# tungphambasement/TNN

Measured on AMD Instinct MI355X. Metric: images/sec (whole node) WRN-16-8 on 32x32x3, pipeline-parallel, higher is better.
Workload: dtype bf16; 1 GPU; model=cifar100_wrn16_8, global_batch=256, input=32x32x3, microbatches=1, graphed_step=True, parallelism=single

## Files before the change

tnn_amd/csrc/bindings.cpp:

```cpp

#include <array>
#include <torch/extension.h>
#include <ATen/hip/HIPContext.h>

#include "kernels.h"

namespace tnn {

static hipStream_t cur_stream() {
  return at::hip::getCurrentHIPStreamMasqueradingAsCUDA().stream();
}

static void* zero_page(const at::Tensor& like) {
  static at::Tensor z;
  if (!z.defined() || z.device() != like.device())
    z = at::zeros({16}, like.options().dtype(at::kFloat));
  return z.data_ptr();
}

static DT dt_of(const at::Tensor& t) {
  if (t.scalar_type() == at::kFloat) return DT::F32;
  if (t.scalar_type() == at::kBFloat16) return DT::BF16;
  TORCH_CHECK(false, "tnn_amd kernels support fp32/bf16, got ", t.scalar_type());
}
// ... 431 lines not shown
at::Tensor conv2d_dgrad(const at::Tensor& dy, const at::Tensor& w, int64_t H,
                        int64_t W, int64_t sh, int64_t sw, int64_t ph,
                        int64_t pw) {
  CHECK_IN(dy);
  CHECK_IN(w);
  int KH = w.size(0), KW = w.size(1), Cin = w.size(2), Cout = w.size(3);
  auto cs = conv_shape_out(dy.size(0), H, W, Cin, Cout, KH, KW, sh, sw, ph, pw,
                           dy.size(1), dy.size(2));
  auto dx = at::empty({cs.N, H, W, Cin}, dy.options());
  if (conv2d_dgrad_wants_db(dt_of(dy), dy.data_ptr(), cs)) {
    auto w_t2d = at::empty({Cin, (int64_t)KH * KW * Cout}, w.options());
    transpose_w_dgrad_launch(dt_of(w), w.data_ptr(), w_t2d.data_ptr(), KH * KW,
                             Cin, Cout, cur_stream());
    conv2d_dgrad_launch(dt_of(dy), dy.data_ptr(), nullptr, w_t2d.data_ptr(),
                        dx.data_ptr(), zero_page(dy), cs, cur_stream());
    return dx;
  }
  auto w_t = at::empty({KH, KW, Cout, Cin}, w.options());
  transpose_w_launch(dt_of(w), w.data_ptr(), w_t.data_ptr(), KH, KW, Cin, Cout,
                     cur_stream());
  conv2d_dgrad_launch(dt_of(dy), dy.data_ptr(), w_t.data_ptr(), nullptr,
                      dx.data_ptr(), zero_page(dy), cs, cur_stream());
  return dx;
}

static at::Tensor conv2d_wgrad_rows(const at::Tensor& x, const at::Tensor& dy,
                                    int64_t KH, int64_t KW, int64_t sh,
                                    int64_t sw, int64_t ph, int64_t pw,
                                    bool out_in_dt, bool bias) {
  CHECK_IN(x);
  CHECK_IN(dy);
  auto cs = conv_shape(x, x.size(3), dy.size(3), KH, KW, sh, sw, ph, pw);
  TORCH_CHECK(dy.size(1) == cs.OH && dy.size(2) == cs.OW, "wgrad shape");
  DT out_dt = out_in_dt ? dt_of(x) : DT::F32;
  const int64_t rows = KH * KW * cs.Cin + (bias ? 1 : 0);
  auto out = at::empty({rows, (int64_t)cs.Cout},
                       out_dt == DT::F32 ? x.options().dtype(at::kFloat)
                                         : x.options());
  int z = conv2d_wgrad_zsplits(cs);
  at::Tensor ws;
  float* wsp = nullptr;
  if (z > 1 || out_dt != DT::F32) {
    ws = at::empty({(int64_t)z * rows * cs.Cout},
                   x.options().dtype(at::kFloat));
    wsp = ws.data_ptr<float>();
  }
// ... 852 lines not shown
  m.def("relu_bwd_mask", &tnn::relu_bwd_mask);
  m.def("add_act_fwd", &tnn::add_act_fwd);
  m.def("add_act_bwd", &tnn::add_act_bwd);
  m.def("dropout_fwd", &tnn::dropout_fwd, py::arg("x"), py::arg("p"),
        py::arg("seed"), py::arg("ctr") = c10::nullopt);
  m.def("dropout_bwd", &tnn::dropout_bwd);
  m.def("colsum", &tnn::colsum);
  m.def("gemm", &tnn::gemm, py::arg("a"), py::arg("b"), py::arg("bias"),
        py::arg("act_kind"), py::arg("residual") = c10::nullopt,
        py::arg("ln_gamma") = c10::nullopt, py::arg("ln_beta") = c10::nullopt,
        py::arg("ln_eps") = 1e-5);
  m.def("gemm_skinny", &tnn::gemm_skinny, py::arg("a"), py::arg("b"),
        py::arg("bias"), py::arg("act_kind"),
        py::arg("residual") = c10::nullopt, py::arg("ln_gamma") = c10::nullopt,
        py::arg("ln_beta") = c10::nullopt, py::arg("ln_eps") = 1e-5);
  m.def("skinny_enabled", &tnn::skinny_enabled);
  m.def("gemm_nt", &tnn::gemm_nt);
  m.def("gemm_tn", &tnn::gemm_tn);
  m.def("mfma_selftest", &tnn::mfma_selftest);
  m.def("mfma_selftest_f32", &tnn::mfma_selftest_f32);
  m.def("conv2d_fwd", &tnn::conv2d_fwd);
  m.def("conv2d_fwd_stats", &tnn::conv2d_fwd_stats);
  m.def("conv2d_dgrad", &tnn::conv2d_dgrad);
  m.def("conv2d_wgrad", &tnn::conv2d_wgrad);
  m.def("conv2d_wgrad_bias", &tnn::conv2d_wgrad_bias);
  m.def("bn_fwd_train", &tnn::bn_fwd_train, py::arg("x"), py::arg("gamma"),
        py::arg("beta"), py::arg("rmean"), py::arg("rvar"),
        py::arg("momentum"), py::arg("eps"), py::arg("relu"),
        py::arg("dropout_p"), py::arg("seed"), py::arg("precomp"),
        py::arg("ctr") = c10::nullopt);
  m.def("bn_fwd_infer", &tnn::bn_fwd_infer);
  m.def("bn_bwd", &tnn::bn_bwd, py::arg("x"), py::arg("dy"),
        py::arg("gamma"), py::arg("mean"), py::arg("invstd"),
        py::arg("y_relu"), py::arg("dy_scale"),
        py::arg("resid") = py::none());
  m.def("maxpool_fwd", &tnn::maxpool_fwd);
  m.def("maxpool_bwd", &tnn::maxpool_bwd);
  m.def("avgpool_fwd", &tnn::avgpool_fwd);
  m.def("avgpool_bwd", &tnn::avgpool_bwd);
  m.def("ce_fwd", &tnn::ce_fwd);
  m.def("ce_bwd", &tnn::ce_bwd);
  m.def("ptloss_fwd", &tnn::ptloss_fwd);
  m.def("ptloss_bwd", &tnn::ptloss_bwd);
  m.def("gn_fwd", &tnn::gn_fwd);
  m.def("gn_bwd", &tnn::gn_bwd);
  m.def("ln_fwd", &tnn::ln_fwd);
// ... 46 lines not shown
```

tnn_amd/csrc/conv2d.hip:

```cpp

#include "common.h"
#include "kernels.h"
#include "tile_gemm.h"

namespace tnn {

using namespace tile;

template <bool POW2>
DEV int idiv(int x, const IDiv& f) {
  if constexpr (POW2) return x >> f.lg;
  else if (f.magic)
    return (int)(((unsigned long long)(unsigned)x * f.magic) >> f.sh);
  else
    return x / f.d;
}
template <bool POW2>
DEV int imod(int x, const IDiv& f) {
  if constexpr (POW2) return x & (f.d - 1);
  else return x - idiv<POW2>(x, f) * f.d;
}

DEV void kdecode(int kidx, const ConvShape& cs, int& kh, int& kw) {
  kh = (kidx * cs.mkw16) >> 16;
// ... 134 lines not shown
    Pack16<T> v = {};
    if (gm < M && gk < K) v = gather(gm, gk);
    *(Pack16<T>*)&As[lds_off<T>(row, kk)] = v;
  }
}
template <typename T, typename RowFn>
DEV void stage_b_transposed(T* Bs, RowFn&& rowptr, int ncols, int n0, int k0,
                            int K) {
  constexpr int V = 16 / sizeof(T);
#pragma unroll
  for (int c = threadIdx.x; c < BK * (BN / V); c += THREADS) {
    int kk = c / (BN / V);
    int nn = (c % (BN / V)) * V;
    int gk = k0 + kk;
    Pack16<T> v = {};
    if (gk < K) v = load16_guarded(rowptr(gk), n0 + nn, ncols);
#pragma unroll
    for (int j = 0; j < V; ++j)
      Bs[lds_off<T>(nn + j, kk)] = v.e[j];
  }
}


template <typename T>
DEV void conv_fwd_store(const WaveCoord& wc, f32x4 acc[FM][FN], const T* bias,
                        T* Y, const ConvShape& cs, int act_kind, int m0,
                        int n0, int M) {
  epilogue_visit(wc, acc, m0, n0, [&](int row, int col, float v) {
    if (row < M && col < cs.Cout) {
      if (bias) v += VecIO<T>::to_f32(bias[col]);
      if (act_kind != ACT_LINEAR) v = act_apply(v, act_kind);
      Y[(int64_t)row * cs.Cout + col] = VecIO<T>::from_f32(v);
    }
  });
}

template <typename T>
DEV void conv_fwd_stats(const WaveCoord& wc, f32x4 acc[FM][FN],
                        const T* bias_p, float* stats, const ConvShape& cs,
                        int m0, int n0, int M) {
  float* ssum = stats;
  float* ssumsq = stats + cs.Cout;
  const int cr = (wc.lane >> 4) * 4;
  const int cc = wc.lane & 15;
#pragma unroll
  for (int fn = 0; fn < FN; ++fn) {
    int col = n0 + wc.wcol0 + fn * 16 + cc;
    float bias = 0.0f;
    if (col < cs.Cout) {
      if (bias_p) bias = VecIO<T>::to_f32(bias_p[col]);
    }
    float s = 0.0f, ss = 0.0f;
#pragma unroll
    for (int fm = 0; fm < FM; ++fm)
#pragma unroll
      for (int j = 0; j < 4; ++j) {
        int row = m0 + wc.wrow0 + fm * 16 + cr + j;
        if (row < M && col < cs.Cout) {
          float v = acc[fm][fn][j] + bias;
          s += v;
          ss += v * v;
        }
      }
    s += __shfl_xor(s, 16, 64);
    ss += __shfl_xor(ss, 16, 64);
    s += __shfl_xor(s, 32, 64);
    ss += __shfl_xor(ss, 32, 64);
    if (wc.lane < 16 && col < cs.Cout) {
      atomicAdd(&ssum[col], s);
      atomicAdd(&ssumsq[col], ss);
    }
  }
}

template <bool POW2, typename T, bool S2>
DEV void dgrad_store(const WaveCoord& wc, f32x4 acc[FM][FN], T* DX,
                     const ConvShape& cs, const DgradClass<S2>& dc, int m0,
                     int n0) {
  epilogue_visit(wc, acc, m0, n0, [&](int row, int col, float v) {
    if (row < dc.M && col < cs.Cin)
      DX[dc.template pixel<POW2>(cs, row) * cs.Cin + col] =
          VecIO<T>::from_f32(v);
  });
}

DEV float* wgrad_slab_store(const WaveCoord& wc, f32x4 acc[FM][FN],
                            float* DW, const ConvShape& cs, int Kout,
                            int bias_row, int r0, int n0) {
  float* out = DW + (int64_t)blockIdx.z * (Kout + bias_row) * cs.Cout;
  epilogue_visit(wc, acc, r0, n0, [&](int row, int col, float v) {
    if (row < Kout && col < cs.Cout) out[(int64_t)row * cs.Cout + col] = v;
  });
  return out;
}
DEV void wgrad_colsum_store(float* out, const ConvShape& cs, int Kout, int n0,
                            float bsum) {
  bsum = colsum_tile_finish(bsum);
  int col = n0 + (threadIdx.x >> 2);
  if ((threadIdx.x & 3) == 0 && col < cs.Cout)
    out[(int64_t)Kout * cs.Cout + col] = bsum;
}

template <bool DB, typename T, typename RowFn, typename TapFn, typename AtFn>
DEV void conv_db_kloop(T* As0, T* As1, T* Bs0, T* Bs1,
                       const WaveCoord& wc, f32x4 acc[FM][FN],
                       const T* __restrict__ asrc, int lgSW, int lgC,
                       const T* __restrict__ bsrc, int64_t bstride,
                       int brows, int m0, int n0, int K,
                       const T* __restrict__ zero16, RowFn&& row,
                       TapFn&& tap, AtFn&& at) {
  constexpr int NA = glds_count<T, BM>();
  constexpr int NB = glds_count<T, BN>();
  constexpr int NPER = NA + NB;
  const int wid = __builtin_amdgcn_readfirstlane(wc.wid);
  const bool uni = lgC >= 6;

  const T* ab[NA];
  int ap[NA], aq[NA];
  const T* bb[NB];
  bool bok[NB];
#pragma unroll
  for (int i = 0; i < NA; ++i) {
    const int j = wid * NA + i;
    int64_t noff;
    int p, q;
    const bool ok = row(m0 + glds_row<T>(j, wc.lane), noff, p, q);
    ab[i] = asrc + noff + (uni ? glds_kk<T>(j, wc.lane) : 0);
    ap[i] = ok ? p : -(1 << 28);
    aq[i] = q;
  }
#pragma unroll
  for (int i = 0; i < NB; ++i) {
    const int j = wid * NB + i;
    const int gn = n0 + glds_row<T>(j, wc.lane);
    bok[i] = gn < brows;
// ... 58 lines not shown
      wait_vmcnt<0>();
    }
    __builtin_amdgcn_s_barrier();
    compute(a_cur, b_cur);
    __builtin_amdgcn_s_barrier();
  };
  if constexpr (DB) {
    stage(0, As0, Bs0);
    for (int t = 0; t < nch; t += 2) {
      step(t, As0, Bs0, As1, Bs1);
      if (t + 1 < nch) step(t + 1, As1, Bs1, As0, Bs0);
    }
  } else {
    for (int t = 0; t < nch; ++t) {
      stage(t, As0, Bs0);
      wait_vmcnt<0>();
      __builtin_amdgcn_s_barrier();
      compute(As0, Bs0);
      __builtin_amdgcn_s_barrier();
    }
  }
}

template <typename T, bool STATS, bool DB>
DEV void conv_fwd_glds_tile(const T* __restrict__ X,
                            const T* __restrict__ WT2,
                            const T* __restrict__ bias, T* __restrict__ Y,
                            const T* __restrict__ zero16, const ConvShape& cs,
                            int act_kind, float* __restrict__ stats) {
  const int M = cs.N * cs.OH * cs.OW;
  const int K = cs.KH * cs.KW * cs.Cin;
  int tm_, tn_;
  conv_tile_order(cs, tm_, tn_);
  const int m0 = tm_ * BM;
  const int n0 = tn_ * BN;
  const WaveCoord wc;
  f32x4 acc[FM][FN] = {};

  auto row = [&](int gm, int64_t& noff, int& p, int& q) {
    const int n = gm >> cs.d_ohow.lg;
    const int rem = gm & (cs.OH * cs.OW - 1);
    p = (rem >> cs.d_ow.lg) * cs.SH - cs.PH;
    q = (rem & (cs.OW - 1)) * cs.SW - cs.PW;
    noff = (int64_t)n << (cs.d_hw.lg + cs.d_cin.lg);
    return gm < M;
  };
  auto tap = [&](int gk, int& dh, int& dw, int& c, int& bcol) {
    kdecode(gk >> cs.d_cin.lg, cs, dh, dw);
    c = gk & (cs.Cin - 1);
    bcol = gk;
  };
  auto at = [&](int p, int q, int dh, int dw, int& ih, int& iw) {
    ih = p + dh;
    iw = q + dw;
    return (unsigned)ih < (unsigned)cs.H && (unsigned)iw < (unsigned)cs.W;
  };
  if constexpr (DB) {
    __shared__ alignas(16) T As0[BM * BK], As1[BM * BK];
    __shared__ alignas(16) T Bs0[BN * BK], Bs1[BN * BK];
    conv_db_kloop<true>(As0, As1, Bs0, Bs1, wc, acc, X, cs.d_w.lg,
                        cs.d_cin.lg, WT2, (int64_t)K, cs.Cout, m0, n0, K,
                        zero16, row, tap, at);
  } else {
    __shared__ alignas(16) T As0[BM * BK], Bs0[BN * BK];
    conv_db_kloop<false>(As0, As0, Bs0, Bs0, wc, acc, X, cs.d_w.lg,
                         cs.d_cin.lg, WT2, (int64_t)K, cs.Cout, m0, n0, K,
                         zero16, row, tap, at);
  }

  conv_fwd_store(wc, acc, bias, Y, cs, act_kind, m0, n0, M);
  if constexpr (STATS) conv_fwd_stats(wc, acc, bias, stats, cs, m0, n0, M);
}

template <typename T, bool STATS = false>
__launch_bounds__(THREADS)
__global__ void k_conv_fwd_db(const T* __restrict__ X,
                              const T* __restrict__ WT2,
                              const T* __restrict__ bias, T* __restrict__ Y,
                              const T* __restrict__ zero16, ConvShape cs,
                              int act_kind, float* __restrict__ stats) {
  conv_fwd_glds_tile<T, STATS, true>(X, WT2, bias, Y, zero16, cs, act_kind,
                                     stats);
}

template <bool STATS>
__launch_bounds__(THREADS)
__global__ void k_conv_fwd_sb(const bf16* __restrict__ X,
                              const bf16* __restrict__ WT2,
                              const bf16* __restrict__ bias,
                              bf16* __restrict__ Y,
                              const bf16* __restrict__ zero16, ConvShape cs,
                              int act_kind, float* __restrict__ stats) {
  conv_fwd_glds_tile<bf16, STATS, false>(X, WT2, bias, Y, zero16, cs, act_kind,
                                         stats);
}

template <typename T, bool POW2, bool GLDS>
__launch_bounds__(THREADS)
__global__ void k_conv_fwd(const T* __restrict__ X, const T* __restrict__ Wt,
                           const T* __restrict__ bias, T* __restrict__ Y,
                           const T* __restrict__ zero16, ConvShape cs,
                           int act_kind) {
  static_assert(!GLDS || POW2, "the LDS-DMA gate implies an all-pow2 shape");
  __shared__ alignas(16) T As[BM * BK];
  __shared__ alignas(16) T Bs[BN * BK];

  const int M = cs.N * cs.OH * cs.OW;
  const int K = cs.KH * cs.KW * cs.Cin;
  int tm_, tn_;
  conv_tile_order(cs, tm_, tn_);
  const int m0 = tm_ * BM;
  const int n0 = tn_ * BN;
  const WaveCoord wc;
  f32x4 acc[FM][FN] = {};

  auto a_src = [&](int k0, int rl, int kk) -> const T* {
    int gm = m0 + rl, gk = k0 + kk;
// ... 68 lines not shown
            if (const T* p = src(gm, gk + j, nullptr)) v.e[j] = *p;
          }
        }
        return v;
      });
    }
    stage_b_transposed(
        Bs,
        [&](int gk) {
          int64_t wrow = gk;
          if constexpr (S2)
            wrow = (int64_t)dc.tap(cs, idiv<POW2>(gk, cs.d_cout)).widx *
                       cs.Cout + imod<POW2>(gk, cs.d_cout);
          return &WT[wrow * cs.Cin];
        },
        cs.Cin, n0, k0, K);
    __syncthreads();
    mfma_compute_tile(As, Bs, wc, acc);
    __syncthreads();
  }
  dgrad_store<POW2>(wc, acc, DX, cs, dc, m0, n0);
}

template <typename T, bool S2 = false, bool S1 = false>
__launch_bounds__(THREADS)
__global__ void k_conv_dgrad_db(const T* __restrict__ DY,
                                const T* __restrict__ WT2D,
                                T* __restrict__ DX,
                                const T* __restrict__ zero16, ConvShape cs) {
  const DgradClass<S2> dc(cs);
  const int M = dc.M, K = dc.K;
  const int KFULL = cs.KH * cs.KW * cs.Cout;
  int tm_, tn_;
  conv_tile_order(cs, tm_, tn_);
  const int m0 = tm_ * BM;
  const int n0 = tn_ * BN;
  const WaveCoord wc;
  f32x4 acc[FM][FN] = {};

  __shared__ alignas(16) T As0[BM * BK], As1[BM * BK];
  __shared__ alignas(16) T Bs0[BN * BK], Bs1[BN * BK];
  conv_db_kloop<true>(
      As0, As1, Bs0, Bs1, wc, acc, DY, cs.d_ow.lg, cs.d_cout.lg, WT2D,
      (int64_t)KFULL, cs.Cin, m0, n0, K, zero16,
      [&](int gm, int64_t& noff, int& p, int& q) {
        const int n = gm >> cs.d_hw.lg;
        const int rem = gm & (dc.Hc * dc.Wc - 1);
        int ih = rem >> cs.d_w.lg, iw = rem & (dc.Wc - 1);
        if constexpr (S2) {
          p = (2 * ih + dc.cls_a + cs.PH - dc.start_h) >> 1;
          q = (2 * iw + dc.cls_b + cs.PW - dc.start_w) >> 1;
        } else {
          p = ih + cs.PH;
          q = iw + cs.PW;
        }
        noff = (int64_t)n << (cs.d_ohow.lg + cs.d_cout.lg);
        return gm < M;
      },
      [&](int gk, int& dh, int& dw, int& c, int& bcol) {
        const int kidx = gk >> cs.d_cout.lg;
        c = gk & (cs.Cout - 1);
        if constexpr (S2) {
          const DgradTap t = dc.tap(cs, kidx);
          dh = t.khi;
          dw = t.kwi;
          bcol = (t.widx << cs.d_cout.lg) + c;
        } else {
          kdecode(kidx, cs, dh, dw);
          bcol = gk;
        }
      },
      [&](int p, int q, int dh, int dw, int& oh, int& ow) {
        const int th = p - dh, tw = q - dw;
        if constexpr (S2 || S1) {
          oh = th;
          ow = tw;
          return (unsigned)oh < (unsigned)cs.OH &&
                 (unsigned)ow < (unsigned)cs.OW;
        } else {
          oh = th / cs.SH;
          ow = tw / cs.SW;
          return th >= 0 && tw >= 0 && oh * cs.SH == th &&
                 ow * cs.SW == tw && oh < cs.OH && ow < cs.OW;
        }
      });
  dgrad_store<true>(wc, acc, DX, cs, dc, m0, n0);
}

template <typename T, bool POW2>
__launch_bounds__(THREADS, 3)
__global__ void k_conv_wgrad(const T* __restrict__ X, const T* __restrict__ DY,
                             float* __restrict__ DW, ConvShape cs,
                             int bias_row) {
  constexpr int V = 16 / sizeof(T);
  __shared__ alignas(16) T As[BM * BK];
  __shared__ alignas(16) T Bs[BN * BK];

  const int M = cs.N * cs.OH * cs.OW;
  const int Kout = cs.KH * cs.KW * cs.Cin;
  int tr_, tn_;
  conv_tile_order(cs, tr_, tn_);
  const int r0 = tr_ * BM;
  const int n0 = tn_ * BN;
  const int m_begin = (int)((int64_t)M * blockIdx.z / gridDim.z);
  const int m_end = (int)((int64_t)M * (blockIdx.z + 1) / gridDim.z);
  const WaveCoord wc;
  f32x4 acc[FM][FN] = {};
  const bool colsum = bias_row && tr_ == 0;
  float bsum = 0.0f;

  for (int k0 = m_begin; k0 < m_end; k0 += BK) {
// ... 274 lines not shown
  return cs.d_ohow.lg >= 0 && cs.d_ow.lg >= 0 && cs.d_cin.lg >= 0 &&
         cs.d_hw.lg >= 0 && cs.d_w.lg >= 0 && cs.d_cout.lg >= 0;
}

static bool vec_ok(DT dt, const void* ptr, int channels) {
  return channels % vec_elems(dt) == 0 && ptr_aligned16(ptr);
}

static int env_int(const char* name, int dflt) {
  const char* e = getenv(name);
  return e ? atoi(e) : dflt;
}

static bool db_on() {
  static const bool on = env_int("TNN_FWD_DB", 1) != 0;
  return on;
}

static int fwd_db_maxk() {
  static const int maxk = env_int("TNN_DB_MAXK", 2304);
  return maxk;
}

template <typename... KArgs, typename... Args>
static void launch(void (*kern)(KArgs...), dim3 grid, hipStream_t s,
                   Args... args) {
  hipLaunchKernelGGL(kern, grid, dim3(THREADS), 0, s, args...);
}

bool conv2d_fwd_wants_db(DT dt, const void* x, const ConvShape& cs) {
  if (!db_on()) return false;
  if (dt == DT::F32 && cs.KH * cs.KW * cs.Cin > fwd_db_maxk()) return false;
  return all_pow2(cs) && vec_ok(dt, x, cs.Cin);
}

static void transpose2d_launch(DT dt, const void* in, void* out, int batch,
                               int rows, int cols, hipStream_t s) {
  dim3 grid((cols + 31) / 32, (rows + 31) / 32, batch);
  dispatch_dt(dt, [&](auto tag) {
    using T = typename decltype(tag)::type;
    hipLaunchKernelGGL(k_transpose2d_tiled<T>, grid, dim3(256), 0, s,
                       (const T*)in, (T*)out, rows, cols);
  });
}

void transpose_w_fwd_launch(DT dt, const void* w, void* w_t2, int KHW, int Cin,
                            int Cout, hipStream_t s) {
  transpose2d_launch(dt, w, w_t2, 1, KHW * Cin, Cout, s);
}

void transpose_w_launch(DT dt, const void* w, void* w_t, int KH, int KW,
                        int Cin, int Cout, hipStream_t s) {
  transpose2d_launch(dt, w, w_t, KH * KW, Cin, Cout, s);
}

void transpose_w_dgrad_launch(DT dt, const void* w, void* w_t2d, int KHW,
                              int Cin, int Cout, hipStream_t s) {
  const bool vec = vec_ok(dt, w, Cout);
  int64_t n = (int64_t)KHW * Cin * (vec ? Cout / vec_elems(dt) : Cout);
  int blocks = (int)((n + 255) / 256);
  dispatch_dt(dt, [&](auto tag) {
    using T = typename decltype(tag)::type;
    auto kern = vec ? k_transpose_w_dgrad_vec<T> : k_transpose_w_dgrad<T>;
    hipLaunchKernelGGL(kern, dim3(blocks), dim3(256), 0, s, (const T*)w,
                       (T*)w_t2d, KHW, Cin, Cout);
  });
}

void conv2d_fwd_launch(DT dt, const void* x, const void* w, const void* w_t2,
                       const void* bias, void* y, const void* zero16,
                       float* stats, const ConvShape& cs, bool relu,
                       hipStream_t s) {
  int M = cs.N * cs.OH * cs.OW;
  dim3 grid(ceil_div(M, BM), ceil_div(cs.Cout, BN));
  int act = relu ? ACT_RELU : ACT_LINEAR;
  bool p2 = all_pow2(cs);
  bool g = p2 && vec_ok(dt, x, cs.Cin);
  dispatch_dt(dt, [&](auto tag) {
    using T = typename decltype(tag)::type;
    auto X = (const T*)x;
    auto B = (const T*)bias;
    auto Y = (T*)y;
    auto Z = (const T*)zero16;
    if (w_t2) {
      if constexpr (sizeof(T) == 2) {
        if (cs.KH * cs.KW * cs.Cin > fwd_db_maxk())
          return launch(stats ? k_conv_fwd_sb<true> : k_conv_fwd_sb<false>,
                        grid, s, X, (const T*)w_t2, B, Y, Z, cs, act, stats);
      }
      return launch(stats ? k_conv_fwd_db<T, true> : k_conv_fwd_db<T, false>,
                    grid, s, X, (const T*)w_t2, B, Y, Z, cs, act, stats);
    }
    launch(g ? k_conv_fwd<T, true, true>
             : (p2 ? k_conv_fwd<T, true, false> : k_conv_fwd<T, false, false>),
           grid, s, X, (const T*)w, B, Y, Z, cs, act);
  });
}

bool conv2d_dgrad_wants_db(DT dt, const void* dy, const ConvShape& cs) {
  if (!db_on()) return false;
  static const int maxk = env_int("TNN_DB_MAXK_DGRAD", 4608);
  return cs.KH * cs.KW * cs.Cout <= maxk && all_pow2(cs) &&
         vec_ok(dt, dy, cs.Cout);
}

void conv2d_dgrad_launch(DT dt, const void* dy, const void* w_t,
                         const void* w_t2d, void* dx, const void* zero16,
                         const ConvShape& cs, hipStream_t s) {
  int M = cs.N * cs.H * cs.W;
  dim3 grid(ceil_div(M, BM), ceil_div(cs.Cin, BN));
  bool p2 = all_pow2(cs);
  bool g = p2 && vec_ok(dt, dy, cs.Cout);
  bool s1 = cs.SH == 1 && cs.SW == 1;
  bool s2 = p2 && cs.SH == 2 && cs.SW == 2 && cs.H % 2 == 0 && cs.W % 2 == 0;
  ConvShape cs2 = cs;
  if (s2) {
    cs2.d_hw.set((cs.H / 2) * (cs.W / 2));
    cs2.d_w.set(cs.W / 2);
    s2 = cs2.d_hw.lg >= 0 && cs2.d_w.lg >= 0;
  }
  dim3 grid_s2(ceil_div(cs.N * (cs.H / 2) * (cs.W / 2), BM),
               ceil_div(cs.Cin, BN), 4);
  dispatch_dt(dt, [&](auto tag) {
    using T = typename decltype(tag)::type;
    auto DY = (const T*)dy;
    auto DX = (T*)dx;
    auto Z = (const T*)zero16;
    if (w_t2d) {
      auto WT = (const T*)w_t2d;
      if (s2)
        return launch(k_conv_dgrad_db<T, true>, grid_s2, s, DY, WT, DX, Z,
                      cs2);
      return launch(s1 ? k_conv_dgrad_db<T, false, true> : k_conv_dgrad_db<T>,
                    grid, s, DY, WT, DX, Z, cs);
    }
    auto WT = (const T*)w_t;
    if (g && s2)
      return launch(k_conv_dgrad<T, true, true, true>, grid_s2, s, DY, WT, DX,
                    Z, cs2);
    launch(g ? (s1 ? k_conv_dgrad<T, true, true, false, true>
                   : k_conv_dgrad<T, true, true>)
             : (p2 ? k_conv_dgrad<T, true, false>
                   : k_conv_dgrad<T, false, false>),
           grid, s, DY, WT, DX, Z, cs);
  });
}

int conv2d_wgrad_zsplits(const ConvShape& cs) {
  int M = cs.N * cs.OH * cs.OW;
  int Kout = cs.KH * cs.KW * cs.Cin;
// ... 40 lines not shown
```

tnn_amd/csrc/kernels.h:

```cpp
#pragma once

#include <hip/hip_runtime.h>
#ifdef __HIPCC__
#include <hip/hip_bf16.h>
#endif
#include <algorithm>
#include <cstdint>

namespace tnn {

enum class DT { F32, BF16 };

inline bool ptr_aligned16(const void* p) { return ((uintptr_t)p & 15) == 0; }

inline int vec_elems(DT dt) { return dt == DT::F32 ? 4 : 8; }

#ifdef __HIPCC__
template <typename T> struct TypeTag { using type = T; };
template <typename F>
inline void dispatch_dt(DT dt, F&& f) {
  if (dt == DT::F32) f(TypeTag<float>{});
  else f(TypeTag<__hip_bfloat16>{});
}
#endif
// ... 84 lines not shown

struct ConvShape {
  int N, H, W, Cin, Cout, KH, KW, SH, SW, PH, PW, OH, OW;
  IDiv d_ohow, d_ow, d_cin, d_hw, d_w, d_cout;
  int mkw16;
  void init_fdiv() {
    d_ohow.set(OH * OW);
    d_ow.set(OW);
    d_cin.set(Cin);
    d_hw.set(H * W);
    d_w.set(W);
    d_cout.set(Cout);
    mkw16 = 65536 / KW + 1;
  }
};
bool conv2d_fwd_wants_db(DT dt, const void* x, const ConvShape& cs);
void transpose_w_fwd_launch(DT dt, const void* w, void* w_t2, int KHW, int Cin,
                            int Cout, hipStream_t s);
void conv2d_fwd_launch(DT dt, const void* x, const void* w, const void* w_t2,
                       const void* bias, void* y, const void* zero16,
                       float* stats, const ConvShape& cs, bool relu,
                       hipStream_t s);
bool conv2d_dgrad_wants_db(DT dt, const void* dy, const ConvShape& cs);
void transpose_w_dgrad_launch(DT dt, const void* w, void* w_t2d, int KHW,
                              int Cin, int Cout, hipStream_t s);
void conv2d_dgrad_launch(DT dt, const void* dy, const void* w_t,
                         const void* w_t2d, void* dx, const void* zero16,
                         const ConvShape& cs, hipStream_t s);
int conv2d_wgrad_zsplits(const ConvShape& cs);
void conv2d_wgrad_launch(DT dt, const void* x, const void* dy, void* dw_out,
                         DT out_dt, float* ws, int z, const void* zero16,
                         const ConvShape& cs, bool bias, hipStream_t s);
void transpose_w_launch(DT dt, const void* w, void* w_t, int KH, int KW,
                        int Cin, int Cout, hipStream_t s);

int64_t bn_stats_ws_floats(DT dt, const void* x, int64_t rows, int cols);
void bn_stats_launch(DT dt, const void* x, float* mean, float* invstd,
                     float* rmean, float* rvar, float momentum, float* ws,
                     int64_t rows, int cols, float eps, hipStream_t s);
void bn_finalize_launch(const float* sum, const float* sumsq, float* mean,
                        float* invstd, float* rmean, float* rvar,
                        float momentum, int64_t rows, int cols, float eps,
                        hipStream_t s);
void bn_apply_launch(DT dt, const void* x, const float* mean,
                     const float* invstd, const float* gamma, const float* beta,
                     void* y, int64_t rows, int cols, bool relu, hipStream_t s);
// ... 145 lines not shown
```

tnn_amd/csrc/tile_gemm.h:

```cpp
#pragma once

#include "common.h"

namespace tile {

constexpr int BM = 128, BN = 64, BK = 64, THREADS = 256;
constexpr int WAVES_M = 2, WAVES_N = 2;
constexpr int WM = BM / WAVES_M;
constexpr int WN = BN / WAVES_N;
constexpr int FM = WM / 16;
constexpr int FN = WN / 16;

template <typename T> struct alignas(16) Pack16 {
  T e[16 / sizeof(T)];
};

template <typename T>
DEV bool aligned16(const T* p) {
  return ((unsigned long long)(const void*)p & 15ull) == 0;
}

template <typename T>
DEV Pack16<T> load16_guarded(const T* row_base, int idx, int limit) {
  constexpr int V = 16 / sizeof(T);
  const T* src = row_base + idx;
  Pack16<T> v = {};
  if (idx + V <= limit && aligned16(src)) {
    v = *(const Pack16<T>*)src;
  } else {
#pragma unroll
    for (int j = 0; j < V; ++j)
      if (idx + j < limit) v.e[j] = src[j];
  }
  return v;
// ... 21 lines not shown
  const int group = id / per_group;
  const int first_m = group * GM;
  const int gm = min(nbx - first_m, GM);
  const int rem = id - group * per_group;
  tm = first_m + rem % gm;
  tn = rem / gm;
}

template <int GM>
DEV void tile_remap_xcd(int& tm, int& tn) {
  const int nbx = gridDim.x, nby = gridDim.y;
  const int T = nbx * nby;
  const int id = blockIdx.y * nbx + blockIdx.x;
  const int lid = (T & 7) == 0 ? ((id & 7) * (T >> 3) + (id >> 3)) : id;
  const int per_group = GM * nby;
  const int group = lid / per_group;
  const int first_m = group * GM;
  const int gm = min(nbx - first_m, GM);
  const int rem = lid - group * per_group;
  tm = first_m + rem % gm;
  tn = rem / gm;
}

struct WaveCoord {
  int wid, lane, wrow0, wcol0;
  DEV WaveCoord() {
    wid = threadIdx.x >> 6;
    lane = threadIdx.x & 63;
    wrow0 = (wid / WAVES_N) * WM;
    wcol0 = (wid % WAVES_N) * WN;
  }
};

template <typename T, int ROWS, typename AddrFn>
DEV void glds_stage(T* As, const WaveCoord& w, AddrFn&& addr) {
  constexpr int ROWB = BK * (int)sizeof(T);
  constexpr int RPK = 1024 / ROWB;
  constexpr int LPR = ROWB / 16;
  constexpr int NREG = ROWS * ROWB / 1024;
  constexpr int NPW = NREG / 4;
#pragma unroll
  for (int i = 0; i < NPW; ++i) {
    const int j = w.wid * NPW + i;
    const int rl = RPK * j + w.lane / LPR;
    const int byte_in_row = (w.lane % LPR) * 16;
    const int kk = (byte_in_row ^ ((((rl >> 3) ^ rl) & 7) << 4)) /
                   (int)sizeof(T);
    const T* src = addr(rl, kk);
    __builtin_amdgcn_global_load_lds(
        (const __attribute__((address_space(1))) unsigned int*)src,
        (__attribute__((address_space(3))) unsigned int*)
            &As[j * (1024 / (int)sizeof(T))],
        16, 0, 0);
  }
}
// ... 62 lines not shown
    for (int fm = 0; fm < FM; ++fm)
#pragma unroll
      for (int fn = 0; fn < FN; ++fn)
        acc[fm][fn] = __builtin_amdgcn_mfma_f32_16x16x4f32(
            a[fm], b[fn], acc[fm][fn], 0, 0, 0);
  }
}

struct RmFrag {
  s16x8 v;
  DEV bf16x8 get() const { return __builtin_bit_cast(bf16x8, v); }
};

DEV RmFrag rm_frag_issue(const bf16* img, int row0, int k0, int lane) {
  typedef __attribute__((address_space(3))) const char* lds_p;
  const unsigned base = (unsigned)(size_t)(lds_p)(const char*)img;
  const int off = lds_off<bf16>(row0 + (lane & 15), k0 + (lane >> 4) * 8);
  RmFrag f;
  asm volatile("ds_read_b128 %0, %1"
               : "=v"(f.v) : "v"(base + 2u * (unsigned)off) : "memory");
  return f;
}

DEV void rm_frags_wait(RmFrag (&a)[FM], RmFrag (&b)[FN]) {
  static_assert(FM == 4 && FN == 2, "operand list below");
  asm volatile("s_waitcnt lgkmcnt(0)"
               : "+v"(a[0].v), "+v"(a[1].v), "+v"(a[2].v), "+v"(a[3].v),
                 "+v"(b[0].v), "+v"(b[1].v)
               :: "memory");
}

DEV void mfma_compute_tile_nofence(const bf16* As, const bf16* Bs,
                                   const WaveCoord& w, f32x4 acc[FM][FN]) {
#pragma unroll
  for (int ks = 0; ks < BK / 32; ++ks) {
    RmFrag a[FM], b[FN];
#pragma unroll
    for (int fm = 0; fm < FM; ++fm)
      a[fm] = rm_frag_issue(As, w.wrow0 + fm * 16, ks * 32, w.lane);
#pragma unroll
    for (int fn = 0; fn < FN; ++fn)
      b[fn] = rm_frag_issue(Bs, w.wcol0 + fn * 16, ks * 32, w.lane);
    rm_frags_wait(a, b);
#pragma unroll
    for (int fm = 0; fm < FM; ++fm)
#pragma unroll
      for (int fn = 0; fn < FN; ++fn)
        acc[fm][fn] = __builtin_amdgcn_mfma_f32_16x16x32_bf16(
            a[fm].get(), b[fn].get(), acc[fm][fn], 0, 0, 0);
  }
}

template <typename T>
DEV int glds_row(int j, int lane) {
  constexpr int ROWB = BK * (int)sizeof(T);
  return (1024 / ROWB) * j + lane / (ROWB / 16);
// ... 81 lines not shown

static_assert(THREADS == 4 * BN, "4 threads per B-tile column");
template <typename T>
DEV float colsum_tile_partial(const T* Bs) {
  constexpr int V = 16 / (int)sizeof(T);
  const int co = threadIdx.x >> 2;
  const int m0 = (threadIdx.x & 3) * (BK / 4);
  float s = 0.0f;
#pragma unroll
  for (int c = 0; c < BK / 4; c += V) {
    Pack16<T> v = *(const Pack16<T>*)&Bs[lds_off<T>(co, m0 + c)];
#pragma unroll
    for (int j = 0; j < V; ++j) s += VecIO<T>::to_f32(v.e[j]);
  }
  return s;
}

DEV float colsum_tile_finish(float s) {
  s += __shfl_xor(s, 1, 64);
  s += __shfl_xor(s, 2, 64);
  return s;
}

template <typename F>
DEV void epilogue_visit(const WaveCoord& w, f32x4 acc[FM][FN],
                        int row0, int col0, F&& emit) {
  const int cr = (w.lane >> 4) * 4;
  const int cc = w.lane & 15;
#pragma unroll
  for (int fm = 0; fm < FM; ++fm)
#pragma unroll
    for (int fn = 0; fn < FN; ++fn)
#pragma unroll
      for (int j = 0; j < 4; ++j) {
        int row = row0 + w.wrow0 + fm * 16 + cr + j;
        int col = col0 + w.wcol0 + fn * 16 + cc;
        emit(row, col, acc[fm][fn][j]);
      }
}

}
```

Baseline: 41060 img/s.

## Add 128x128 wide-tile bf16 conv fwd/dgrad kernels with route selection

```diff
diff --git a/tnn_amd/csrc/bindings.cpp b/tnn_amd/csrc/bindings.cpp
--- a/tnn_amd/csrc/bindings.cpp
+++ b/tnn_amd/csrc/bindings.cpp
@@ -477,6 +477,27 @@
   conv2d_dgrad_launch(dt_of(dy), dy.data_ptr(), w_t.data_ptr(), nullptr,
                       dx.data_ptr(), zero_page(dy), cs, cur_stream());
   return dx;
+}
+
+std::string conv2d_fwd_route_name(const at::Tensor& x, const at::Tensor& w,
+                                  int64_t sh, int64_t sw, int64_t ph,
+                                  int64_t pw, bool stats) {
+  CHECK_IN(x);
+  CHECK_IN(w);
+  auto cs = conv_shape(x, w.size(2), w.size(3), w.size(0), w.size(1), sh, sw,
+                       ph, pw);
+  return conv2d_fwd_route(dt_of(x), x.data_ptr(), cs, stats);
+}
+
+std::string conv2d_dgrad_route_name(const at::Tensor& dy,
+                                    const at::Tensor& w, int64_t H, int64_t W,
+                                    int64_t sh, int64_t sw, int64_t ph,
+                                    int64_t pw) {
+  CHECK_IN(dy);
+  CHECK_IN(w);
+  auto cs = conv_shape_out(dy.size(0), H, W, w.size(2), w.size(3), w.size(0),
+                           w.size(1), sh, sw, ph, pw, dy.size(1), dy.size(2));
+  return conv2d_dgrad_route(dt_of(dy), dy.data_ptr(), cs);
 }
 
 static at::Tensor conv2d_wgrad_rows(const at::Tensor& x, const at::Tensor& dy,
@@ -1375,6 +1396,8 @@
   m.def("conv2d_fwd", &tnn::conv2d_fwd);
   m.def("conv2d_fwd_stats", &tnn::conv2d_fwd_stats);
   m.def("conv2d_dgrad", &tnn::conv2d_dgrad);
+  m.def("conv2d_fwd_route", &tnn::conv2d_fwd_route_name);
+  m.def("conv2d_dgrad_route", &tnn::conv2d_dgrad_route_name);
   m.def("conv2d_wgrad", &tnn::conv2d_wgrad);
   m.def("conv2d_wgrad_bias", &tnn::conv2d_wgrad_bias);
   m.def("bn_fwd_train", &tnn::bn_fwd_train, py::arg("x"), py::arg("gamma"),
diff --git a/tnn_amd/csrc/conv2d.hip b/tnn_amd/csrc/conv2d.hip
--- a/tnn_amd/csrc/conv2d.hip
+++ b/tnn_amd/csrc/conv2d.hip
@@ -180,10 +180,10 @@
 }
 
 
-template <typename T>
-DEV void conv_fwd_store(const WaveCoord& wc, f32x4 acc[FM][FN], const T* bias,
-                        T* Y, const ConvShape& cs, int act_kind, int m0,
-                        int n0, int M) {
+template <typename T, typename S>
+DEV void conv_fwd_store(const WaveCoordT<S>& wc, f32x4 acc[S::FM][S::FN],
+                        const T* bias, T* Y, const ConvShape& cs, int act_kind,
+                        int m0, int n0, int M) {
   epilogue_visit(wc, acc, m0, n0, [&](int row, int col, float v) {
     if (row < M && col < cs.Cout) {
       if (bias) v += VecIO<T>::to_f32(bias[col]);
@@ -193,10 +193,11 @@
   });
 }
 
-template <typename T>
-DEV void conv_fwd_stats(const WaveCoord& wc, f32x4 acc[FM][FN],
+template <typename T, typename S>
+DEV void conv_fwd_stats(const WaveCoordT<S>& wc, f32x4 acc[S::FM][S::FN],
                         const T* bias_p, float* stats, const ConvShape& cs,
                         int m0, int n0, int M) {
+  constexpr int FM = S::FM, FN = S::FN;
   float* ssum = stats;
   float* ssumsq = stats + cs.Cout;
   const int cr = (wc.lane >> 4) * 4;
@@ -231,8 +232,8 @@
   }
 }
 
-template <bool POW2, typename T, bool S2>
-DEV void dgrad_store(const WaveCoord& wc, f32x4 acc[FM][FN], T* DX,
+template <bool POW2, typename T, bool S2, typename S>
+DEV void dgrad_store(const WaveCoordT<S>& wc, f32x4 acc[S::FM][S::FN], T* DX,
                      const ConvShape& cs, const DgradClass<S2>& dc, int m0,
                      int n0) {
   epilogue_visit(wc, acc, m0, n0, [&](int row, int col, float v) {
@@ -259,16 +260,17 @@
     out[(int64_t)Kout * cs.Cout + col] = bsum;
 }
 
-template <bool DB, typename T, typename RowFn, typename TapFn, typename AtFn>
+template <bool DB, typename T, typename S, typename RowFn, typename TapFn,
+          typename AtFn>
 DEV void conv_db_kloop(T* As0, T* As1, T* Bs0, T* Bs1,
-                       const WaveCoord& wc, f32x4 acc[FM][FN],
+                       const WaveCoordT<S>& wc, f32x4 acc[S::FM][S::FN],
                        const T* __restrict__ asrc, int lgSW, int lgC,
                        const T* __restrict__ bsrc, int64_t bstride,
                        int brows, int m0, int n0, int K,
                        const T* __restrict__ zero16, RowFn&& row,
                        TapFn&& tap, AtFn&& at) {
-  constexpr int NA = glds_count<T, BM>();
-  constexpr int NB = glds_count<T, BN>();
+  constexpr int NA = glds_count<T, S::BM>();
+  constexpr int NB = glds_count<T, S::BN>();
   constexpr int NPER = NA + NB;
   const int wid = __builtin_amdgcn_readfirstlane(wc.wid);
   const bool uni = lgC >= 6;
@@ -373,7 +375,7 @@
   }
 }
 
-template <typename T, bool STATS, bool DB>
+template <typename T, bool STATS, bool DB, typename S = TileStd>
 DEV void conv_fwd_glds_tile(const T* __restrict__ X,
                             const T* __restrict__ WT2,
                             const T* __restrict__ bias, T* __restrict__ Y,
@@ -383,10 +385,10 @@
   const int K = cs.KH * cs.KW * cs.Cin;
   int tm_, tn_;
   conv_tile_order(cs, tm_, tn_);
-  const int m0 = tm_ * BM;
-  const int n0 = tn_ * BN;
-  const WaveCoord wc;
-  f32x4 acc[FM][FN] = {};
+  const int m0 = tm_ * S::BM;
+  const int n0 = tn_ * S::BN;
+  const WaveCoordT<S> wc;
+  f32x4 acc[S::FM][S::FN] = {};
 
   auto row = [&](int gm, int64_t& noff, int& p, int& q) {
     const int n = gm >> cs.d_ohow.lg;
@@ -407,13 +409,13 @@
     return (unsigned)ih < (unsigned)cs.H && (unsigned)iw < (unsigned)cs.W;
   };
   if constexpr (DB) {
-    __shared__ alignas(16) T As0[BM * BK], As1[BM * BK];
-    __shared__ alignas(16) T Bs0[BN * BK], Bs1[BN * BK];
+    __shared__ alignas(16) T As0[S::BM * BK], As1[S::BM * BK];
+    __shared__ alignas(16) T Bs0[S::BN * BK], Bs1[S::BN * BK];
     conv_db_kloop<true>(As0, As1, Bs0, Bs1, wc, acc, X, cs.d_w.lg,
                         cs.d_cin.lg, WT2, (int64_t)K, cs.Cout, m0, n0, K,
                         zero16, row, tap, at);
   } else {
-    __shared__ alignas(16) T As0[BM * BK], Bs0[BN * BK];
+    __shared__ alignas(16) T As0[S::BM * BK], Bs0[S::BN * BK];
     conv_db_kloop<false>(As0, As0, Bs0, Bs0, wc, acc, X, cs.d_w.lg,
                          cs.d_cin.lg, WT2, (int64_t)K, cs.Cout, m0, n0, K,
                          zero16, row, tap, at);
@@ -444,6 +446,31 @@
                               int act_kind, float* __restrict__ stats) {
   conv_fwd_glds_tile<bf16, STATS, false>(X, WT2, bias, Y, zero16, cs, act_kind,
                                          stats);
+}
+
+template <bool STATS>
+__launch_bounds__(THREADS, 2)
+__global__ void k_conv_fwd_db_wide(const bf16* __restrict__ X,
+                                   const bf16* __restrict__ WT2,
+                                   const bf16* __restrict__ bias,
+                                   bf16* __restrict__ Y,
+                                   const bf16* __restrict__ zero16,
+                                   ConvShape cs, int act_kind,
+                                   float* __restrict__ stats) {
+  conv_fwd_glds_tile<bf16, STATS, true, TileWide>(X, WT2, bias, Y, zero16, cs,
+                                                  act_kind, stats);
+}
+template <bool STATS>
+__launch_bounds__(THREADS, 3)
+__global__ void k_conv_fwd_sb_wide(const bf16* __restrict__ X,
+                                   const bf16* __restrict__ WT2,
+                                   const bf16* __restrict__ bias,
+                                   bf16* __restrict__ Y,
+                                   const bf16* __restrict__ zero16,
+                                   ConvShape cs, int act_kind,
+                                   float* __restrict__ stats) {
+  conv_fwd_glds_tile<bf16, STATS, false, TileWide>(X, WT2, bias, Y, zero16, cs,
+                                                   act_kind, stats);
 }
 
 template <typename T, bool POW2, bool GLDS>
@@ -558,25 +585,22 @@
   dgrad_store<POW2>(wc, acc, DX, cs, dc, m0, n0);
 }
 
-template <typename T, bool S2 = false, bool S1 = false>
-__launch_bounds__(THREADS)
-__global__ void k_conv_dgrad_db(const T* __restrict__ DY,
-                                const T* __restrict__ WT2D,
-                                T* __restrict__ DX,
-                                const T* __restrict__ zero16, ConvShape cs) {
+template <typename T, bool S2, bool S1, bool DB, typename S = TileStd>
+DEV void conv_dgrad_glds_tile(const T* DY, const T* WT2D, T* DX,
+                              const T* zero16, const ConvShape& cs) {
   const DgradClass<S2> dc(cs);
   const int M = dc.M, K = dc.K;
   const int KFULL = cs.KH * cs.KW * cs.Cout;
   int tm_, tn_;
   conv_tile_order(cs, tm_, tn_);
-  const int m0 = tm_ * BM;
-  const int n0 = tn_ * BN;
-  const WaveCoord wc;
-  f32x4 acc[FM][FN] = {};
-
-  __shared__ alignas(16) T As0[BM * BK], As1[BM * BK];
-  __shared__ alignas(16) T Bs0[BN * BK], Bs1[BN * BK];
-  conv_db_kloop<true>(
+  const int m0 = tm_ * S::BM;
+  const int n0 = tn_ * S::BN;
+  const WaveCoordT<S> wc;
+  f32x4 acc[S::FM][S::FN] = {};
+
+  __shared__ alignas(16) T As0[S::BM * BK], As1[DB ? S::BM * BK : 8];
+  __shared__ alignas(16) T Bs0[S::BN * BK], Bs1[DB ? S::BN * BK : 8];
+  conv_db_kloop<DB>(
       As0, As1, Bs0, Bs1, wc, acc, DY, cs.d_ow.lg, cs.d_cout.lg, WT2D,
       (int64_t)KFULL, cs.Cin, m0, n0, K, zero16,
       [&](int gm, int64_t& noff, int& p, int& q) {
@@ -623,6 +647,35 @@
   dgrad_store<true>(wc, acc, DX, cs, dc, m0, n0);
 }
 
+template <typename T, bool S2 = false, bool S1 = false>
+__launch_bounds__(THREADS)
+__global__ void k_conv_dgrad_db(const T* __restrict__ DY,
+                                const T* __restrict__ WT2D,
+                                T* __restrict__ DX,
+                                const T* __restrict__ zero16, ConvShape cs) {
+  conv_dgrad_glds_tile<T, S2, S1, true>(DY, WT2D, DX, zero16, cs);
+}
+
+template <bool S2 = false, bool S1 = false>
+__launch_bounds__(THREADS, 2)
+__global__ void k_conv_dgrad_db_wide(const bf16* __restrict__ DY,
+                                     const bf16* __restrict__ WT2D,
+                                     bf16* __restrict__ DX,
+                                     const bf16* __restrict__ zero16,
+                                     ConvShape cs) {
+  conv_dgrad_glds_tile<bf16, S2, S1, true, TileWide>(DY, WT2D, DX, zero16, cs);
+}
+template <bool S2 = false, bool S1 = false>
+__launch_bounds__(THREADS, 3)
+__global__ void k_conv_dgrad_sb_wide(const bf16* __restrict__ DY,
+                                     const bf16* __restrict__ WT2D,
+                                     bf16* __restrict__ DX,
+                                     const bf16* __restrict__ zero16,
+                                     ConvShape cs) {
+  conv_dgrad_glds_tile<bf16, S2, S1, false, TileWide>(DY, WT2D, DX, zero16,
+                                                      cs);
+}
+
 template <typename T, bool POW2>
 __launch_bounds__(THREADS, 3)
 __global__ void k_conv_wgrad(const T* __restrict__ X, const T* __restrict__ DY,
@@ -943,6 +996,43 @@
   return maxk;
 }
 
+static int wide_mode() {
+  static const int mode = env_int("TNN_CONV_WIDE", 1);
+  return mode;
+}
+static int wide_buf() {
+  static const int buf = env_int("TNN_CONV_WIDE_BUF", 0);
+  return buf;
+}
+
+enum class Wide { NO, DB, SB };
+constexpr int WIDE_MIN_TILES = 512;
+constexpr int WIDE_FWD_DB_MINK = 2048;
+constexpr int WIDE_DGRAD_SB_MAXK = 1152;
+static Wide wide_pick(bool eligible, int tiles, bool take, bool single) {
+  if (!eligible || wide_mode() == 0) return Wide::NO;
+  if (wide_mode() == 1 && !(take && tiles >= WIDE_MIN_TILES)) return Wide::NO;
+  if (wide_buf() != 0) single = wide_buf() == 2;
+  return single ? Wide::SB : Wide::DB;
+}
+static Wide fwd_wide(DT dt, bool have_wt2, const ConvShape& cs, bool stats) {
+  const int nt = cs.Cout / TileWide::BN;
+  const int K = cs.KH * cs.KW * cs.Cin;
+  const bool take = nt == 1 ? !stats : K >= WIDE_FWD_DB_MINK;
+  return wide_pick(
+      have_wt2 && dt == DT::BF16 && cs.Cout % TileWide::BN == 0,
+      ceil_div(cs.N * cs.OH * cs.OW, TileWide::BM) * nt, take, nt == 1);
+}
+static Wide dgrad_wide(DT dt, bool have_wt2d, bool s2, const ConvShape& cs) {
+  const int M = s2 ? cs.N * (cs.H / 2) * (cs.W / 2) : cs.N * cs.H * cs.W;
+  const int taps =
+      s2 ? ((cs.KH + 1) / 2) * ((cs.KW + 1) / 2) : cs.KH * cs.KW;
+  return wide_pick(
+      have_wt2d && dt == DT::BF16 && cs.Cin % TileWide::BN == 0,
+      ceil_div(M, TileWide::BM) * (cs.Cin / TileWide::BN) * (s2 ? 4 : 1),
+      true, taps * cs.Cout <= WIDE_DGRAD_SB_MAXK);
+}
+
 template <typename... KArgs, typename... Args>
 static void launch(void (*kern)(KArgs...), dim3 grid, hipStream_t s,
                    Args... args) {
@@ -988,32 +1078,71 @@
   });
 }
 
+enum class FwdRoute { SB_WIDE, DB_WIDE, SB, DB, GLDS, POW2, GENERIC };
+static FwdRoute fwd_route(DT dt, const void* x, bool have_wt2,
+                          const ConvShape& cs, bool stats) {
+  if (have_wt2) {
+    const Wide wide = fwd_wide(dt, true, cs, stats);
+    if (wide != Wide::NO)
+      return wide == Wide::SB ? FwdRoute::SB_WIDE : FwdRoute::DB_WIDE;
+    const bool long_k =
+        dt == DT::BF16 && cs.KH * cs.KW * cs.Cin > fwd_db_maxk();
+    return long_k ? FwdRoute::SB : FwdRoute::DB;
+  }
+  if (!all_pow2(cs)) return FwdRoute::GENERIC;
+  return vec_ok(dt, x, cs.Cin) ? FwdRoute::GLDS : FwdRoute::POW2;
+}
+
+const char* conv2d_fwd_route(DT dt, const void* x, const ConvShape& cs,
+                             bool stats) {
+  const bool db = conv2d_fwd_wants_db(dt, x, cs);
+  switch (fwd_route(dt, x, db, cs, db && stats)) {
+    case FwdRoute::SB_WIDE: return "k_conv_fwd_sb_wide";
+    case FwdRoute::DB_WIDE: return "k_conv_fwd_db_wide";
+    case FwdRoute::SB: return "k_conv_fwd_sb";
+    case FwdRoute::DB: return "k_conv_fwd_db";
+    case FwdRoute::GLDS: return "k_conv_fwd<pow2, glds>";
+    case FwdRoute::POW2: return "k_conv_fwd<pow2>";
+    default: return "k_conv_fwd";
+  }
+}
+
 void conv2d_fwd_launch(DT dt, const void* x, const void* w, const void* w_t2,
                        const void* bias, void* y, const void* zero16,
                        float* stats, const ConvShape& cs, bool relu,
                        hipStream_t s) {
   int M = cs.N * cs.OH * cs.OW;
   dim3 grid(ceil_div(M, BM), ceil_div(cs.Cout, BN));
+  dim3 grid_wide(ceil_div(M, TileWide::BM), ceil_div(cs.Cout, TileWide::BN));
   int act = relu ? ACT_RELU : ACT_LINEAR;
-  bool p2 = all_pow2(cs);
-  bool g = p2 && vec_ok(dt, x, cs.Cin);
+  const FwdRoute route =
+      fwd_route(dt, x, w_t2 != nullptr, cs, stats != nullptr);
   dispatch_dt(dt, [&](auto tag) {
     using T = typename decltype(tag)::type;
     auto X = (const T*)x;
     auto B = (const T*)bias;
     auto Y = (T*)y;
     auto Z = (const T*)zero16;
-    if (w_t2) {
-      if constexpr (sizeof(T) == 2) {
-        if (cs.KH * cs.KW * cs.Cin > fwd_db_maxk())
-          return launch(stats ? k_conv_fwd_sb<true> : k_conv_fwd_sb<false>,
-                        grid, s, X, (const T*)w_t2, B, Y, Z, cs, act, stats);
-      }
+    if constexpr (sizeof(T) == 2) {
+      if (route == FwdRoute::SB_WIDE)
+        return launch(
+            stats ? k_conv_fwd_sb_wide<true> : k_conv_fwd_sb_wide<false>,
+            grid_wide, s, X, (const T*)w_t2, B, Y, Z, cs, act, stats);
+      if (route == FwdRoute::DB_WIDE)
+        return launch(
+            stats ? k_conv_fwd_db_wide<true> : k_conv_fwd_db_wide<false>,
+            grid_wide, s, X, (const T*)w_t2, B, Y, Z, cs, act, stats);
+      if (route == FwdRoute::SB)
+        return launch(stats ? k_conv_fwd_sb<true> : k_conv_fwd_sb<false>,
+                      grid, s, X, (const T*)w_t2, B, Y, Z, cs, act, stats);
+    }
+    if (route == FwdRoute::DB)
       return launch(stats ? k_conv_fwd_db<T, true> : k_conv_fwd_db<T, false>,
                     grid, s, X, (const T*)w_t2, B, Y, Z, cs, act, stats);
-    }
-    launch(g ? k_conv_fwd<T, true, true>
-             : (p2 ? k_conv_fwd<T, true, false> : k_conv_fwd<T, false, false>),
+    launch(route == FwdRoute::GLDS
+               ? k_conv_fwd<T, true, true>
+               : (route == FwdRoute::POW2 ? k_conv_fwd<T, true, false>
+                                          : k_conv_fwd<T, false, false>),
            grid, s, X, (const T*)w, B, Y, Z, cs, act);
   });
 }
@@ -1023,6 +1152,41 @@
   static const int maxk = env_int("TNN_DB_MAXK_DGRAD", 4608);
   return cs.KH * cs.KW * cs.Cout <= maxk && all_pow2(cs) &&
          vec_ok(dt, dy, cs.Cout);
+}
+
+static bool dgrad_parity(const ConvShape& cs, ConvShape& cs2) {
+  bool s2 = all_pow2(cs) && cs.SH == 2 && cs.SW == 2 && cs.H % 2 == 0 &&
+            cs.W % 2 == 0;
+  cs2 = cs;
+  if (s2) {
+    cs2.d_hw.set((cs.H / 2) * (cs.W / 2));
+    cs2.d_w.set(cs.W / 2);
+    s2 = cs2.d_hw.lg >= 0 && cs2.d_w.lg >= 0;
+  }
+  return s2;
+}
+
+const char* conv2d_dgrad_route(DT dt, const void* dy, const ConvShape& cs) {
+  ConvShape cs2;
+  const bool s2 = dgrad_parity(cs, cs2);
+  const bool s1 = cs.SH == 1 && cs.SW == 1;
+  const bool p2 = all_pow2(cs);
+  if (conv2d_dgrad_wants_db(dt, dy, cs)) {
+    const Wide wide = dgrad_wide(dt, true, s2, cs);
+    if (wide == Wide::SB)
+      return s2 ? "k_conv_dgrad_sb_wide<S2>"
+                : (s1 ? "k_conv_dgrad_sb_wide<S1>" : "k_conv_dgrad_sb_wide");
+    if (wide == Wide::DB)
+      return s2 ? "k_conv_dgrad_db_wide<S2>"
+                : (s1 ? "k_conv_dgrad_db_wide<S1>" : "k_conv_dgrad_db_wide");
+    return s2 ? "k_conv_dgrad_db<S2>"
+              : (s1 ? "k_conv_dgrad_db<S1>" : "k_conv_dgrad_db");
+  }
+  if (p2 && vec_ok(dt, dy, cs.Cout))
+    return s2 ? "k_conv_dgrad<pow2, glds, S2>"
+              : (s1 ? "k_conv_dgrad<pow2, glds, S1>"
+                    : "k_conv_dgrad<pow2, glds>");
+  return p2 ? "k_conv_dgrad<pow2>" : "k_conv_dgrad";
 }
 
 void conv2d_dgrad_launch(DT dt, const void* dy, const void* w_t,
@@ -1033,20 +1197,35 @@
   bool p2 = all_pow2(cs);
   bool g = p2 && vec_ok(dt, dy, cs.Cout);
   bool s1 = cs.SH == 1 && cs.SW == 1;
-  bool s2 = p2 && cs.SH == 2 && cs.SW == 2 && cs.H % 2 == 0 && cs.W % 2 == 0;
-  ConvShape cs2 = cs;
-  if (s2) {
-    cs2.d_hw.set((cs.H / 2) * (cs.W / 2));
-    cs2.d_w.set(cs.W / 2);
-    s2 = cs2.d_hw.lg >= 0 && cs2.d_w.lg >= 0;
-  }
-  dim3 grid_s2(ceil_div(cs.N * (cs.H / 2) * (cs.W / 2), BM),
-               ceil_div(cs.Cin, BN), 4);
+  ConvShape cs2;
+  bool s2 = dgrad_parity(cs, cs2);
+  int Mc = cs.N * (cs.H / 2) * (cs.W / 2);
+  dim3 grid_s2(ceil_div(Mc, BM), ceil_div(cs.Cin, BN), 4);
+  const Wide wide = dgrad_wide(dt, w_t2d != nullptr, s2, cs);
   dispatch_dt(dt, [&](auto tag) {
     using T = typename decltype(tag)::type;
     auto DY = (const T*)dy;
     auto DX = (T*)dx;
     auto Z = (const T*)zero16;
+    if constexpr (sizeof(T) == 2) {
+      if (wide != Wide::NO) {
+        auto WT = (const T*)w_t2d;
+        constexpr int WBM = TileWide::BM, WBN = TileWide::BN;
+        const bool sb = wide == Wide::SB;
+        if (s2)
+          return launch(sb ? k_conv_dgrad_sb_wide<true>
+                           : k_conv_dgrad_db_wide<true>,
+                        dim3(ceil_div(Mc, WBM), cs.Cin / WBN, 4), s, DY, WT,
+                        DX, Z, cs2);
+        dim3 gw(ceil_div(M, WBM), cs.Cin / WBN);
+        if (s1)
+          return launch(sb ? k_conv_dgrad_sb_wide<false, true>
+                           : k_conv_dgrad_db_wide<false, true>,
+                        gw, s, DY, WT, DX, Z, cs);
+        return launch(sb ? k_conv_dgrad_sb_wide<> : k_conv_dgrad_db_wide<>,
+                      gw, s, DY, WT, DX, Z, cs);
+      }
+    }
     if (w_t2d) {
       auto WT = (const T*)w_t2d;
       if (s2)
diff --git a/tnn_amd/csrc/kernels.h b/tnn_amd/csrc/kernels.h
--- a/tnn_amd/csrc/kernels.h
+++ b/tnn_amd/csrc/kernels.h
@@ -130,6 +130,9 @@
                        float* stats, const ConvShape& cs, bool relu,
                        hipStream_t s);
 bool conv2d_dgrad_wants_db(DT dt, const void* dy, const ConvShape& cs);
+const char* conv2d_fwd_route(DT dt, const void* x, const ConvShape& cs,
+                             bool stats);
+const char* conv2d_dgrad_route(DT dt, const void* dy, const ConvShape& cs);
 void transpose_w_dgrad_launch(DT dt, const void* w, void* w_t2d, int KHW,
                               int Cin, int Cout, hipStream_t s);
 void conv2d_dgrad_launch(DT dt, const void* dy, const void* w_t,
diff --git a/tnn_amd/csrc/tile_gemm.h b/tnn_amd/csrc/tile_gemm.h
--- a/tnn_amd/csrc/tile_gemm.h
+++ b/tnn_amd/csrc/tile_gemm.h
@@ -4,12 +4,28 @@
 
 namespace tile {
 
-constexpr int BM = 128, BN = 64, BK = 64, THREADS = 256;
-constexpr int WAVES_M = 2, WAVES_N = 2;
-constexpr int WM = BM / WAVES_M;
-constexpr int WN = BN / WAVES_N;
-constexpr int FM = WM / 16;
-constexpr int FN = WN / 16;
+constexpr int BK = 64, THREADS = 256;
+
+template <int BM_, int BN_, int WAVES_M_ = 2, int WAVES_N_ = 2>
+struct TileShape {
+  static constexpr int BM = BM_, BN = BN_;
+  static constexpr int WAVES_M = WAVES_M_, WAVES_N = WAVES_N_;
+  static constexpr int WM = BM / WAVES_M;
+  static constexpr int WN = BN / WAVES_N;
+  static constexpr int FM = WM / 16;
+  static constexpr int FN = WN / 16;
+  static_assert(WAVES_M * WAVES_N * 64 == THREADS, "one wave per sub-tile");
+  static_assert(WM % 16 == 0 && WN % 16 == 0, "whole 16x16 fragments");
+};
+using TileStd = TileShape<128, 64>;
+using TileWide = TileShape<128, 128>;
+
+constexpr int BM = TileStd::BM, BN = TileStd::BN;
+constexpr int WAVES_M = TileStd::WAVES_M, WAVES_N = TileStd::WAVES_N;
+constexpr int WM = TileStd::WM;
+constexpr int WN = TileStd::WN;
+constexpr int FM = TileStd::FM;
+constexpr int FN = TileStd::FN;
 
 template <typename T> struct alignas(16) Pack16 {
   T e[16 / sizeof(T)];
@@ -77,15 +93,18 @@
   tn = rem / gm;
 }
 
-struct WaveCoord {
+template <typename S = TileStd>
+struct WaveCoordT {
+  using Shape = S;
   int wid, lane, wrow0, wcol0;
-  DEV WaveCoord() {
+  DEV WaveCoordT() {
     wid = threadIdx.x >> 6;
     lane = threadIdx.x & 63;
-    wrow0 = (wid / WAVES_N) * WM;
-    wcol0 = (wid % WAVES_N) * WN;
-  }
-};
+    wrow0 = (wid / S::WAVES_N) * S::WM;
+    wcol0 = (wid % S::WAVES_N) * S::WN;
+  }
+};
+using WaveCoord = WaveCoordT<>;
 
 template <typename T, int ROWS, typename AddrFn>
 DEV void glds_stage(T* As, const WaveCoord& w, AddrFn&& addr) {
@@ -194,16 +213,26 @@
   return f;
 }
 
-DEV void rm_frags_wait(RmFrag (&a)[FM], RmFrag (&b)[FN]) {
-  static_assert(FM == 4 && FN == 2, "operand list below");
-  asm volatile("s_waitcnt lgkmcnt(0)"
-               : "+v"(a[0].v), "+v"(a[1].v), "+v"(a[2].v), "+v"(a[3].v),
-                 "+v"(b[0].v), "+v"(b[1].v)
-               :: "memory");
-}
-
+template <int NFM, int NFN>
+DEV void rm_frags_wait(RmFrag (&a)[NFM], RmFrag (&b)[NFN]) {
+  static_assert(NFM == 4 && (NFN == 2 || NFN == 4), "operand lists below");
+  if constexpr (NFN == 2)
+    asm volatile("s_waitcnt lgkmcnt(0)"
+                 : "+v"(a[0].v), "+v"(a[1].v), "+v"(a[2].v), "+v"(a[3].v),
+                   "+v"(b[0].v), "+v"(b[1].v)
+                 :: "memory");
+  else
+    asm volatile("s_waitcnt lgkmcnt(0)"
+                 : "+v"(a[0].v), "+v"(a[1].v), "+v"(a[2].v), "+v"(a[3].v),
+                   "+v"(b[0].v), "+v"(b[1].v), "+v"(b[2].v), "+v"(b[3].v)
+                 :: "memory");
+}
+
+template <typename S>
 DEV void mfma_compute_tile_nofence(const bf16* As, const bf16* Bs,
-                                   const WaveCoord& w, f32x4 acc[FM][FN]) {
+                                   const WaveCoordT<S>& w,
+                                   f32x4 acc[S::FM][S::FN]) {
+  constexpr int FM = S::FM, FN = S::FN;
 #pragma unroll
   for (int ks = 0; ks < BK / 32; ++ks) {
     RmFrag a[FM], b[FN];
@@ -331,9 +360,10 @@
   return s;
 }
 
-template <typename F>
-DEV void epilogue_visit(const WaveCoord& w, f32x4 acc[FM][FN],
+template <typename S, typename F>
+DEV void epilogue_visit(const WaveCoordT<S>& w, f32x4 acc[S::FM][S::FN],
                         int row0, int col0, F&& emit) {
+  constexpr int FM = S::FM, FN = S::FN;
   const int cr = (w.lane >> 4) * 4;
   const int cc = w.lane & 15;
 #pragma unroll
```

Result: faster. 42920 img/s, median of 6 (+4.5%).
